# zuds-survey/zuds-pipeline

Hardware: AMD Instinct MI355X
Metric: Mpix/s resample->coadd->subtract, 3072x3072 frames (higher is better)
Workload: dtype f32; 1 GPU; configs[1]+[2]: 32x 3072x3072 TPV frames/GPU, mesh background + weight rescale + Lanczos-3 resample + WEIGHTED coadd (+ AND mask coadd, int16 masks); then 1 science frame/GPU: align ref, hotpants 3x3 regions x 10x10 stamps, r=10, ko=4, subtract; frames_per_gpu=32, size=3072, mask_dtype=int16, combine=WEIGHTED, subtract=True

## Files before the change

### zuds-pipeline_amd/csrc/hotpants.hip

```cpp
#include "hp_dev.h"
#include <sched.h>
#include "chol_diag.h"

__global__ void k_hp_valid(const float* __restrict__ sci, const float* __restrict__ ref,
                           const uint8_t* __restrict__ bpm, int64_t n, float il, float iu,
                           float tl, float tu, uint8_t* __restrict__ bad,
                           const double* __restrict__ lim, double nsig) {
    int64_t p = (int64_t)blockIdx.x * blockDim.x + threadIdx.x;
    if (lim) {
        il = (float)(lim[0] - nsig * lim[1]);
        tl = (float)(lim[3] - nsig * lim[4]);
    }
    if (p >= n) return;
    float s = sci[p], t = ref[p];
    bool ok = (s == s) && (t == t) && fabsf(s) < 3e38f && fabsf(t) < 3e38f;
    ok = ok && s >= il && s <= iu && t >= tl && t <= tu;
    if (bpm) ok = ok && bpm[p] == 0;
    bad[p] = ok ? 0 : 1;
}

#define HP_ROWMAX 16384
__global__ __launch_bounds__(256) void k_hp_rowany(const uint8_t* __restrict__ in, int nx, int ny, int hw,
                                                   uint8_t* __restrict__ out) {
    extern __shared__ int ra_pre[];
// ... 1811 lines not shown
    if (tid < 64) {
        auto run_chain = [&](double* xout) {
            const int li = tid & 31;
            double col[CH_NB];
#pragma unroll
            for (int j = 0; j < CH_NB; ++j) col[j] = Dn[j][li];
            const double rdl = Dn[li][CH_NB];
            double u = ys[li];
#pragma unroll
            for (int j = 1; j < CH_NB; ++j) col[j] *= readlane_d(rdl, j);
#pragma unroll
            for (int j = CH_NB - 1; j >= 1; --j) u = __builtin_fma(-col[j], readlane_d(u, j), u);
            if (tid < CH_NB) xout[tid] = u * rdl;
        };
        __syncthreads();
        run_chain(xs[0]);
        __syncthreads();
        for (int kb = nblk - 1; kb >= 1; --kb) {
            __syncthreads();
            run_chain(xs[(nblk - kb) & 1]);
            __syncthreads();
        }
        return;
    }
    const int c = tid - 64;
    double yc = 0.0, a[CH_NB], dnext[2] = {0.0, 0.0};
    auto diag_elem = [&](int k0, int nb, int e) -> double {
        const int i = e >> 5, j = e & 31;
        return (i < nb && j <= i) ? A[(size_t)(k0 + i) * lda + k0 + j] : (i == j ? 1.0 : 0.0);
    };
    auto diag_put = [&](int e, double v) {
        const int i = e >> 5, j = e & 31;
        Dn[i][j] = (i == j) ? 0.0 : v;
        if (i == j) Dn[i][CH_NB] = 1.0 / v;
    };
    {
        const int kb = nblk - 1, k0 = kb * CH_NB, nb = n - k0;
        yc = (c < n) ? A[(size_t)n * lda + c] : 0.0;
        diag_put(c, diag_elem(k0, nb, c));
        if (c + CBC_COLS < CH_NB * CH_NB) diag_put(c + CBC_COLS, diag_elem(k0, nb, c + CBC_COLS));
        if (c >= k0 && c < k0 + CH_NB) ys[c - k0] = yc;
#pragma unroll
        for (int m = 0; m < CH_NB; ++m) a[m] = (c < k0 && m < nb) ? A[(size_t)(k0 + m) * lda + c] : 0.0;
        if (kb > 0) {
            dnext[0] = diag_elem(k0 - CH_NB, CH_NB, c);
            if (c + CBC_COLS < CH_NB * CH_NB) dnext[1] = diag_elem(k0 - CH_NB, CH_NB, c + CBC_COLS);
        }
    }
    __syncthreads();
    __syncthreads();
    for (int kb = nblk - 1; kb >= 1; --kb) {
        const int k0 = kb * CH_NB, nb = min(CH_NB, n - k0);
        const int k0n = k0 - CH_NB;
        const double* xc = xs[(nblk - 1 - kb) & 1];
        if (c >= k0 && c < k0 + nb) yc = xc[c - k0];
        if (c >= k0n && c < k0) {
            double acc = 0.0;
#pragma unroll
            for (int m = 0; m < CH_NB; ++m) acc += a[m] * xc[m];
            yc -= acc;
            ys[c - k0n] = yc;
        }
        diag_put(c, dnext[0]);
        if (c + CBC_COLS < CH_NB * CH_NB) diag_put(c + CBC_COLS, dnext[1]);
        __syncthreads();
        if (c < k0n) {
            double acc = 0.0;
#pragma unroll
            for (int m = 0; m < CH_NB; ++m) acc += a[m] * xc[m];
            yc -= acc;
        }
#pragma unroll
        for (int m = 0; m < CH_NB; ++m) a[m] = (c < k0n) ? A[(size_t)(k0n + m) * lda + c] : 0.0;
        if (kb > 1) {
            dnext[0] = diag_elem(k0n - CH_NB, CH_NB, c);
            if (c + CBC_COLS < CH_NB * CH_NB) dnext[1] = diag_elem(k0n - CH_NB, CH_NB, c + CBC_COLS);
        }
        __syncthreads();
    }
    if (c < min(CH_NB, n)) yc = xs[(nblk - 1) & 1][c];
    if (c < n) xall[(size_t)blockIdx.x * n + c] = yc / dall[(size_t)blockIdx.x * n + c];
}

static __device__ __forceinline__ void hp_merit_body(const hp_plan& P, const double* __restrict__ G,
                                                 const double* __restrict__ phi,
                                                 const double* __restrict__ vbar,
                                                 const int* __restrict__ active,
                                                 const double* __restrict__ xsol,
                                                 double* __restrict__ merit, const int* __restrict__ guard,
                                                 int* __restrict__ needlist) {
    if (guard && *guard == 0) return;
    __shared__ double c[HP_MAXX];
    const int cell = blockIdx.x, lane = threadIdx.x;
    if (needlist && cell == 0 && lane == 0) needlist[0] = 0;
    if (active[cell] < 0) { if (lane == 0) merit[cell] = -1.0; return; }
    const int reg = cell / P.ncellr;
    const double* x = xsol + (size_t)reg * P.nunk;
    const double* ph = phi + (size_t)cell * P.nkp;
    const double* Gc = G + (size_t)cell * HP_MAXX * HP_MAXX;
    if (lane < P.nE) {
        double v;
        if (lane == 0) v = x[0];
        else if (lane < P.nc) {
            v = 0.0;
            for (int p = 0; p < P.nkp; ++p) v += x[1 + (lane - 1) * P.nkp + p] * ph[p];
        } else v = x[1 + (P.nc - 1) * P.nkp + (lane - P.nc)];
        c[lane] = v;
    }
    __syncthreads();
    double part = 0.0;
    if (lane < P.nE) {
        double q = 0.0;
        for (int m = 0; m < P.nE; ++m) q += Gc[lane * HP_MAXX + m] * c[m];
        part = c[lane] * (q - 2.0 * Gc[lane * HP_MAXX + P.nE]);
    }
    part = wave_sum_d(part);
    if (lane == 0) merit[cell] = (Gc[P.nE * HP_MAXX + P.nE] + part) / (P.npix * vbar[cell]);
}

#define HP_RFLAG_TMO (1 << 30)
#define HP_RFLAG_DONE 0x80000000u
struct hp_sig {
    int* done;
    unsigned long long* host;
    unsigned seq;
};
static __device__ __forceinline__ void hp_round_signal(const hp_sig& sg, int* round_flag, int nblocks) {
    if (!sg.host) return;
    __threadfence();
    __syncthreads();
    if (threadIdx.x == 0 && atomicAdd(sg.done, 1) == nblocks - 1) {
        const unsigned v = (unsigned)atomicAdd(round_flag, 0);
        __threadfence_system();
        __hip_atomic_store(sg.host, ((unsigned long long)sg.seq << 32) | v | HP_RFLAG_DONE, __ATOMIC_RELEASE,
                           __HIP_MEMORY_SCOPE_SYSTEM);
    }
}
__global__ __launch_bounds__(256) void k_hp_reject(const hp_plan P, const double* __restrict__ merit,
                                                   const int2* __restrict__ centres,
                                                   int* __restrict__ active, int* __restrict__ need,
                                                   int* __restrict__ chg, int* __restrict__ nrej,
                                                   double* __restrict__ stats, const int* __restrict__ guard, int* __restrict__ round_flag,
                                                   int* __restrict__ needlist, const int* __restrict__ tmo = nullptr,
                                                   const hp_sig sig = hp_sig{nullptr, nullptr, 0u}) {
    if (guard && *guard == 0) {
        hp_round_signal(sig, round_flag, gridDim.x);
        return;
    }
    __shared__ double red[4];
    const int reg = blockIdx.x, tid = threadIdx.x;
    double m = 0.0, s = 0.0;
    for (int pass = 0; pass < 4; ++pass) {
        double s0 = 0, s1 = 0;
        for (int k = tid; k < P.ncellr; k += 256) {
            double v = merit[reg * P.ncellr + k];
            if (active[reg * P.ncellr + k] < 0) continue;
            if (pass == 0 || fabs(v - m) <= 3.0 * s) { s0 += 1.0; s1 += v; }
        }
        s0 = block_sum256(s0, red);
        s1 = block_sum256(s1, red);
        if (s0 < 1.0) break;
        double mn = s1 / s0, s2 = 0;
        for (int k = tid; k < P.ncellr; k += 256) {
            double v = merit[reg * P.ncellr + k];
            if (active[reg * P.ncellr + k] < 0) continue;
            if (pass == 0 || fabs(v - m) <= 3.0 * s) s2 += (v - mn) * (v - mn);
        }
        s2 = block_sum256(s2, red);
        m = mn;
        s = sqrt(s2 / s0);
    }
    const double lim = m + P.ks * s;
    double cnt = 0, msum = 0, used = 0;
    for (int k = tid; k < P.ncellr; k += 256) {
        const int cell = reg * P.ncellr + k;
        int a = active[cell];
        need[cell] = 0;
        chg[cell] = 0;
        if (a < 0) continue;
        double v = merit[cell];
        used += 1.0;
        msum += v;
        if (v > lim) {
            cnt += 1.0;
            a += 1;
            if (a >= P.nss || centres[cell * P.nss + a].x < 0) a = -1;
            else {
                need[cell] = 1;
                if (needlist) needlist[1 + atomicAdd(&needlist[0], 1)] = cell;
            }
            active[cell] = a;
            chg[cell] = 1;
        }
    }
    cnt = block_sum256(cnt, red);
    msum = block_sum256(msum, red);
    used = block_sum256(used, red);
    if (tid == 0) {
        nrej[reg] = (int)cnt;
        if (cnt > 0) atomicAdd(round_flag, (int)cnt);
        if (tmo && tmo[reg]) atomicOr(round_flag, HP_RFLAG_TMO);
        stats[reg * 2 + 0] = used > 0 ? msum / used : 0.0;
        stats[reg * 2 + 1] = used;
    }
    __syncthreads();
    if (tid == 0) {
        int* list = chg + P.ncell + reg * (P.ncellr + 1);
        int k = 0;
        for (int c = 0; c < P.ncellr; ++c)
            if (chg[reg * P.ncellr + c]) list[1 + k++] = reg * P.ncellr + c;
        list[0] = k;
    }
    hp_round_signal(sig, round_flag, gridDim.x);
}

static __device__ __forceinline__ void hp_reject_wave_body(const hp_plan& P, const double* __restrict__ merit,
                                                       const int2* __restrict__ centres,
                                                       int* __restrict__ active, int* __restrict__ need,
                                                       int* __restrict__ chg, int* __restrict__ nrej,
                                                       double* __restrict__ stats, const int* __restrict__ guard,
                                                       int* __restrict__ round_flag, int* __restrict__ needlist,
                                                       const int* __restrict__ tmo = nullptr) {
    if (guard && *guard == 0) return;
    const int reg = blockIdx.x, lane = threadIdx.x;
    double mv[4];
    int av[4];
#pragma unroll
    for (int u = 0; u < 4; ++u) {
        const int k = lane + 64 * u;
        mv[u] = k < P.ncellr ? merit[reg * P.ncellr + k] : 0.0;
        av[u] = k < P.ncellr ? active[reg * P.ncellr + k] : -1;
    }
    double m = 0.0, s = 0.0;
    for (int pass = 0; pass < 4; ++pass) {
        double s0 = 0, s1 = 0;
#pragma unroll
        for (int u = 0; u < 4; ++u)
            if (av[u] >= 0 && (pass == 0 || fabs(mv[u] - m) <= 3.0 * s)) { s0 += 1.0; s1 += mv[u]; }
        s0 = wave_sum_d(s0);
        s1 = wave_sum_d(s1);
        if (s0 < 1.0) break;
        const double mn = s1 / s0;
        double s2 = 0;
#pragma unroll
        for (int u = 0; u < 4; ++u)
            if (av[u] >= 0 && (pass == 0 || fabs(mv[u] - m) <= 3.0 * s)) s2 += (mv[u] - mn) * (mv[u] - mn);
        s2 = wave_sum_d(s2);
        m = mn;
        s = sqrt(s2 / s0);
    }
    const double lim = m + P.ks * s;
    double cnt = 0, msum = 0, used = 0;
    unsigned long long chm[4];
#pragma unroll
    for (int u = 0; u < 4; ++u) {
        const int k = lane + 64 * u;
        bool changed = false;
        if (k < P.ncellr) {
            const int cell = reg * P.ncellr + k;
            int a = av[u];
            int nd = 0;
            if (a >= 0) {
                used += 1.0;
                msum += mv[u];
                if (mv[u] > lim) {
                    cnt += 1.0;
                    a += 1;
                    if (a >= P.nss || centres[cell * P.nss + a].x < 0) a = -1;
                    else nd = 1;
                    active[cell] = a;
                    changed = true;
                }
            }
            need[cell] = nd;
            chg[cell] = changed ? 1 : 0;
            if (nd && needlist) needlist[1 + atomicAdd(&needlist[0], 1)] = cell;
        }
        chm[u] = __ballot(changed);
    }
    cnt = wave_sum_d(cnt);
    msum = wave_sum_d(msum);
    used = wave_sum_d(used);
    if (lane == 0) {
        nrej[reg] = (int)cnt;
        if (cnt > 0) atomicAdd(round_flag, (int)cnt);
        if (tmo && tmo[reg]) atomicOr(round_flag, HP_RFLAG_TMO);
        stats[reg * 2 + 0] = used > 0 ? msum / used : 0.0;
        stats[reg * 2 + 1] = used;
    }
    int* list = chg + P.ncell + reg * (P.ncellr + 1);
    int base = 0;
#pragma unroll
    for (int u = 0; u < 4; ++u) {
        const unsigned long long bm = chm[u];
        if (bm >> lane & 1ull)
            list[1 + base + __popcll(bm & ((1ull << lane) - 1ull))] = reg * P.ncellr + lane + 64 * u;
        base += __popcll(bm);
    }
    if (lane == 0) list[0] = base;
}

__global__ void k_hp_init_active(const hp_plan P, const int2* __restrict__ centres,
                                 int* __restrict__ active, int* __restrict__ need,
                                 int* __restrict__ ntotal) {
    int cell = blockIdx.x * blockDim.x + threadIdx.x;
    if (cell >= P.ncell) return;
    bool has = centres[cell * P.nss].x >= 0;
    active[cell] = has ? 0 : -1;
    need[cell] = has ? 1 : 0;
    if (has) atomicAdd(&ntotal[cell / P.ncellr], 1);
}

__global__ __launch_bounds__(256) void k_hp_gram(const hp_plan P, const double* __restrict__ X,
// ... 72 lines not shown
}

__global__ void k_hp_scale(int n, int lda, const double* __restrict__ A0, const double* __restrict__ rhs0,
                           double* __restrict__ A, const double* __restrict__ d, unsigned* __restrict__ bar,
                           const int* __restrict__ guard, unsigned* __restrict__ dff, int ndff) {
    hp_scale_body(blockIdx.z, n, lda, A0, rhs0, A, d, bar, guard, dff, ndff);
}
#define HSB_ROWS 8
__global__ __launch_bounds__(256) void k_hp_scale_b(int n, int lda, int nreg, const hp_job* __restrict__ jobs, int round,
                                                    int ncell, int ncellr) {
    const hp_job& J = jobs[blockIdx.y / nreg];
    const int* guard = HPJ_GUARD(J, round);
    if (guard && *guard == 0) return;
    const int reg = blockIdx.y % nreg;
    if (HPJ_REGION_IDLE(J, round, reg, ncell, ncellr)) return;
    const double* __restrict__ dd = J.dsc + (size_t)reg * n;
    const double* __restrict__ A0 = J.A0 + (size_t)reg * (size_t)(n + 1) * n;
    const double* __restrict__ rhs0 = J.rhs0 + (size_t)reg * n;
    double* __restrict__ A = J.A + (size_t)reg * (size_t)(n + 1) * lda;
#pragma unroll 1
    for (int k = 0; k < HSB_ROWS; ++k) {
        const int c1 = blockIdx.x * HSB_ROWS + k;
        if (c1 >= n) break;
        const double r1 = 1.0 / dd[c1];
        for (int c2 = threadIdx.x; c2 <= c1; c2 += 256) {
            const double r2 = 1.0 / dd[c2];
            double v = __dmul_rn(A0[(size_t)c1 * n + c2], __dmul_rn(r1, r2));
            if (c1 == c2) v = __dadd_rn(v, HP_RIDGE);
            A[(size_t)c1 * lda + c2] = v;
        }
        if (threadIdx.x == 0) A[(size_t)n * lda + c1] = __dmul_rn(rhs0[c1], r1);
    }
}

__global__ __launch_bounds__(CT_THREADS) void k_chol_tp(int n, int lda, int ldt, double* Aall, double* ATall, int* fail,
                                                        long long* prof, const int* __restrict__ guard) {
    chol_tp_body(n, lda, ldt, Aall, ATall, fail, prof, guard);
}
__global__ __launch_bounds__(CT_THREADS) void k_chol_tp_b(int n, int lda, int ldt, const hp_job* __restrict__ jobs, int round,
                                                          int ncell, int ncellr) {
    const hp_job& J = jobs[blockIdx.z];
    if (HPJ_REGION_IDLE(J, round, (int)blockIdx.x, ncell, ncellr)) return;
    chol_tp_body(n, lda, ldt, J.A, J.AT, HPJ_FAIL(J), nullptr, HPJ_GUARD(J, round));
}

__global__ __launch_bounds__(CBC_THREADS) void k_chol_back_cols(int n, int lda, const double* __restrict__ Aall,
                                                                const double* __restrict__ dall,
                                                                double* __restrict__ xall, const int* __restrict__ guard) {
    chol_back_cols_body(n, lda, Aall, dall, xall, guard);
}
__global__ __launch_bounds__(CBC_THREADS) void k_chol_back_cols_b(int n, int lda, const hp_job* __restrict__ jobs, int round,
                                                                  int ncell, int ncellr) {
    const hp_job& J = jobs[blockIdx.z];
    if (HPJ_REGION_IDLE(J, round, (int)blockIdx.x, ncell, ncellr)) return;
    chol_back_cols_body(n, lda, J.A, J.dsc, J.rhs, HPJ_GUARD(J, round));
}

__global__ __launch_bounds__(64) void k_hp_merit(const hp_plan P, const double* __restrict__ G,
                                                 const double* __restrict__ phi, const double* __restrict__ vbar,
                                                 const int* __restrict__ active, const double* __restrict__ xsol,
                                                 double* __restrict__ merit, const int* __restrict__ guard,
                                                 int* __restrict__ needlist) {
    hp_merit_body(P, G, phi, vbar, active, xsol, merit, guard, needlist);
}
__global__ __launch_bounds__(64) void k_hp_merit_b(const hp_plan P, const hp_job* __restrict__ jobs, int round) {
    const hp_job& J = jobs[blockIdx.z];
    hp_merit_body(P, J.G, J.phi, J.vbar, J.active, J.rhs, J.merit, HPJ_GUARD(J, round), J.needlist);
}

__global__ __launch_bounds__(64) void k_hp_reject_wave(const hp_plan P, const double* __restrict__ merit,
                                                       const int2* __restrict__ centres, int* __restrict__ active,
                                                       int* __restrict__ need, int* __restrict__ chg,
                                                       int* __restrict__ nrej, double* __restrict__ stats,
                                                       const int* __restrict__ guard, int* __restrict__ round_flag,
                                                       int* __restrict__ needlist, const int* __restrict__ tmo,
                                                       const hp_sig sig) {
    hp_reject_wave_body(P, merit, centres, active, need, chg, nrej, stats, guard, round_flag, needlist, tmo);
    hp_round_signal(sig, round_flag, gridDim.x);
}
__global__ __launch_bounds__(64) void k_hp_reject_wave_b(const hp_plan P, const hp_job* __restrict__ jobs, int round) {
    const hp_job& J = jobs[blockIdx.z];
    hp_reject_wave_body(P, J.merit, J.centres, J.active, J.need, J.chg, HPJ_NREJ(J), J.stats, HPJ_GUARD(J, round),
                        J.rflags + round, J.needlist);
}

__global__ void k_hp_flag(int32_t* __restrict__ mask, const float* __restrict__ img, float value, int32_t bit,
                          int64_t n, const int* __restrict__ tmo, int nreg) {
    int gaveup = 0;
    for (int r = 0; r < nreg; ++r) gaveup |= tmo[r];
    if (gaveup) return;
    int64_t p = (int64_t)blockIdx.x * blockDim.x + threadIdx.x;
    if (p >= n) return;
    if (img[p] == value) mask[p] |= bit;
}

extern "C" void zm_hp_params_default(zm_hp_params* p) {
    if (!p) return;
    memset(p, 0, sizeof(*p));
    p->tu = 5e3; p->tl = 0.0; p->iu = 5e3; p->il = 0.0;
    p->r = 10.0; p->rss = 15.0;
    p->fin = sqrt(50000.0); p->fi = 1e-30;
    p->nsx = p->nsy = 10; p->nrx = p->nry = 1;
    p->ko = 4; p->bgo = 0; p->nss = 3; p->normalize = 0;
    p->ft = 20.0; p->ks = 2.0;
    p->ngauss = 3;
    p->deg[0] = 6; p->deg[1] = 4; p->deg[2] = 2;
    p->sigma[0] = 0.7; p->sigma[1] = 1.5; p->sigma[2] = 3.0;
    p->limits_dev = nullptr; p->limits_nsigma = 10.0;
}

static int make_plan(const zm_hp_params* hp, int nx, int ny, hp_plan* P, std::vector<double>* filt,
                     std::vector<double>* basis) {
    memset(P, 0, sizeof(*P));
    P->nx = nx; P->ny = ny;
    P->hwk = (int)hp->r; P->hwss = (int)hp->rss;
    ZM_CHECK(P->hwk >= 1 && P->hwk <= HP_MAX_HWK, "zm_subtract: kernel half width int(r) = %d outside [1, %d]", P->hwk, HP_MAX_HWK);
    ZM_CHECK(P->hwss >= 1 && P->hwss <= HP_MAX_HWSS, "zm_subtract: substamp half width int(rss) = %d outside [1, %d]", P->hwss, HP_MAX_HWSS);
    P->hw = P->hwk + P->hwss;
    P->step = 2 * P->hwk + 1; P->sw = 2 * P->hwss + 1; P->pw = 2 * P->hw + 1;
    P->npix = P->sw * P->sw;
    P->npixp = (P->npix + GR_KT - 1) / GR_KT * GR_KT;
    ZM_CHECK(hp->ngauss >= 1 && hp->ngauss <= 4, "zm_subtract: ngauss %d outside [1, 4]", hp->ngauss);
    ZM_CHECK(hp->ko >= 0 && hp->ko <= 6, "zm_subtract: -ko %d outside [0, 6]", hp->ko);
    ZM_CHECK(hp->bgo >= 0 && hp->bgo <= 3, "zm_subtract: -bgo %d outside [0, 3]", hp->bgo);
    ZM_CHECK(hp->nss >= 1 && hp->nss <= HP_MAXNSS, "zm_subtract: nss %d outside [1, %d]", hp->nss, HP_MAXNSS);
    ZM_CHECK(hp->nrx >= 1 && hp->nry >= 1 && hp->nrx * hp->nry <= HP_MAXREG, "zm_subtract: bad -nrx/-nry");
    ZM_CHECK(hp->nsx >= 1 && hp->nsy >= 1 && hp->nsx * hp->nsy <= 4096, "zm_subtract: bad -nsx/-nsy");
    P->ko = hp->ko; P->bgo = hp->bgo; P->nss = hp->nss; P->normalize = hp->normalize;
    P->nrx = hp->nrx; P->nry = hp->nry; P->nsx = hp->nsx; P->nsy = hp->nsy;
    P->nreg = hp->nrx * hp->nry; P->ncellr = hp->nsx * hp->nsy; P->ncell = P->nreg * P->ncellr;
    P->tu = hp->tu; P->tl = hp->tl; P->iu = hp->iu; P->il = hp->il; P->ft = hp->ft; P->ks = hp->ks;
    P->fi = (float)hp->fi; P->fin = (float)hp->fin;
    ZM_CHECK(nx / hp->nrx / hp->nsx >= 1 && ny / hp->nry / hp->nsy >= 1, "zm_subtract: stamps smaller than a pixel");
    for (int ry = 0; ry < hp->nry; ++ry)
        for (int rx = 0; rx < hp->nrx; ++rx) {
            int r = ry * hp->nrx + rx;
            P->rx0[r] = rx * (nx / hp->nrx);
            P->rx1[r] = rx == hp->nrx - 1 ? nx : (rx + 1) * (nx / hp->nrx);
            P->ry0[r] = ry * (ny / hp->nry);
            P->ry1[r] = ry == hp->nry - 1 ? ny : (ry + 1) * (ny / hp->nry);
        }
    const int step = P->step, hwk = P->hwk;
    std::vector<int> fidx;
    int nf1 = 0, nc = 0;
    std::vector<double> fsum;
    filt->clear();
    int base[4] = {0, 0, 0, 0};
    for (int g = 0; g < hp->ngauss; ++g) {
        ZM_CHECK(hp->deg[g] >= 0 && hp->deg[g] <= 8 && hp->sigma[g] > 0, "zm_subtract: bad basis");
        base[g] = nf1;
        P->gdeg[g] = hp->deg[g];
        P->gbase[g] = nf1;
        for (int a = 0; a <= hp->deg[g]; ++a) {
            double s = 0.0;
            for (int u = -hwk; u <= hwk; ++u) {
                double v = exp(-(double)u * u / (2.0 * hp->sigma[g] * hp->sigma[g])) * pow((double)u, (double)a);
                filt->push_back(v);
                s += v;
            }
            fsum.push_back(s);
            ++nf1;
        }
    }
    ZM_CHECK(nf1 <= HP_MAXF1, "zm_subtract: too many 1-D filters");
    P->nf1 = nf1;
    P->ngauss = hp->ngauss;
// ... 189 lines not shown
    ZM_TRY(ctx->get("hp_bad", np, (void**)&bad));
    ZM_TRY(ctx->get("hp_tmp8", np, (void**)&tmp8));
    ZM_TRY(ctx->get("hp_dirty", np, (void**)&dirty));
    ZM_TRY(ctx->get("hp_outbad", np, (void**)&outbad));
    int2* centres = nullptr;
    int *active = nullptr, *need = nullptr, *ibuf = nullptr;
    double *X = nullptr, *G = nullptr, *phi = nullptr, *vbar = nullptr, *A = nullptr, *rhs = nullptr,
           *dsc = nullptr, *merit = nullptr, *stats = nullptr, *d_filt = nullptr;
    ZM_TRY(ctx->get("hp_centres", sizeof(int2) * P.ncell * P.nss, (void**)&centres));
    ZM_TRY(ctx->get("hp_active", sizeof(int) * P.ncell, (void**)&active));
    ZM_TRY(ctx->get("hp_need", sizeof(int) * P.ncell, (void**)&need));
    int* needlist = nullptr;
    ZM_TRY(ctx->get("hp_needlist", sizeof(int) * ((size_t)P.ncell + 1), (void**)&needlist));
    int* chg = nullptr;
    ZM_TRY(ctx->get("hp_chg", sizeof(int) * (2 * (size_t)P.ncell + P.nreg), (void**)&chg));
    constexpr int HP_NIBUF = 4 * HP_MAXREG + 4;
    constexpr size_t HP_SUMBYTES = sizeof(int) * HP_NIBUF + sizeof(double) * 3 * HP_MAXREG;
    static_assert((sizeof(int) * HP_NIBUF) % 8 == 0, "the statistics behind the counters are doubles");
    char* sumbuf = nullptr;
    ZM_TRY(ctx->get("hp_summary", HP_SUMBYTES, (void**)&sumbuf));
    ibuf = reinterpret_cast<int*>(sumbuf);
    int *nrej = ibuf, *ntotal = ibuf + HP_MAXREG, *fail = ibuf + 2 * HP_MAXREG, *nmasked = ibuf + 3 * HP_MAXREG;
    int* tmo = ibuf + 3 * HP_MAXREG + 4;
    unsigned* cbar = nullptr;
    ZM_TRY(ctx->get("hp_cbar", sizeof(unsigned) * CF_BAR_STRIDE * HP_MAXREG, (void**)&cbar));
    double* cdg = nullptr;
    ZM_TRY(ctx->get("hp_cdg", sizeof(double) * 4 * CH_NB * (CH_NB + 1) * HP_MAXREG, (void**)&cdg));
    ZM_TRY(ctx->get("hp_X", sizeof(double) * (size_t)P.ncell * P.nX * P.npixp, (void**)&X));
    ZM_TRY(ctx->get("hp_G", sizeof(double) * (size_t)P.ncell * HP_MAXX * HP_MAXX, (void**)&G));
    double* Gp = nullptr;
    ZM_TRY(ctx->get("hp_Gp", sizeof(double) * (size_t)P.ncell * GR_SPLIT * HP_MAXX * HP_MAXX, (void**)&Gp));
    ZM_TRY(ctx->get("hp_phi", sizeof(double) * (size_t)P.ncell * P.nkp, (void**)&phi));
    double *Gold = nullptr, *phiold = nullptr;
    ZM_TRY(ctx->get("hp_Gold", sizeof(double) * (size_t)P.ncell * HP_MAXX * HP_MAXX, (void**)&Gold));
    ZM_TRY(ctx->get("hp_phiold", sizeof(double) * (size_t)P.ncell * P.nkp, (void**)&phiold));
    ZM_TRY(ctx->get("hp_vbar", sizeof(double) * P.ncell, (void**)&vbar));
    const int lda = (P.nunk + 15) & ~15;
    ZM_TRY(ctx->get("hp_A", sizeof(double) * (size_t)P.nreg * (P.nunk + 1) * lda, (void**)&A));
    ZM_TRY(ctx->get("hp_rhs", sizeof(double) * (size_t)P.nreg * P.nunk, (void**)&rhs));
    double *A0 = nullptr, *rhs0 = nullptr;
    ZM_TRY(ctx->get("hp_A0", sizeof(double) * (size_t)P.nreg * (P.nunk + 1) * P.nunk, (void**)&A0));
    ZM_TRY(ctx->get("hp_rhs0", sizeof(double) * (size_t)P.nreg * P.nunk, (void**)&rhs0));
    ZM_TRY(ctx->get("hp_dsc", sizeof(double) * (size_t)P.nreg * P.nunk, (void**)&dsc));
    ZM_TRY(ctx->get("hp_merit", sizeof(double) * P.ncell, (void**)&merit));
    stats = reinterpret_cast<double*>(sumbuf + sizeof(int) * HP_NIBUF);
    double* x0sum = stats + 2 * HP_MAXREG;
    ZM_TRY(ctx->get("hp_filt", sizeof(double) * filt.size(), (void**)&d_filt));
    if (!(ctx->hp_filt_dev == (const void*)d_filt && ctx->hp_filt_host == filt)) {
        double* h_tab = nullptr;
        ZM_TRY(ctx->get_pinned("hp_tab", sizeof(double) * filt.size(), (void**)&h_tab));
        ZM_HIP(hipStreamSynchronize(st));
        memcpy(h_tab, filt.data(), sizeof(double) * filt.size());
        ZM_HIP(hipMemcpyAsync(d_filt, h_tab, sizeof(double) * filt.size(), hipMemcpyHostToDevice, st));
        ctx->hp_filt_host = filt;
        ctx->hp_filt_dev = d_filt;
    }

    const dim3 b256(256);
    ZM_TRY(hp_launch_masks(ctx, P, hp, sci, ref, bpm, bad, tmp8, dirty, outbad));
    char* h_sum = nullptr;
    ZM_TRY(ctx->get_pinned("hp_summary_h", HP_SUMBYTES, (void**)&h_sum));
    const int* h_int = reinterpret_cast<const int*>(h_sum);
    const double* h_stats = reinterpret_cast<const double*>(h_sum + sizeof(int) * HP_NIBUF);
    const double* h_x0 = h_stats + 2 * HP_MAXREG;
    int rounds = 0, retries = 0, ntimeouts = 0;
    const char* spin_env = getenv("ZM_CHOL_SPIN_LIMIT");
    hp_fit_guard fitting(&g_hp_fitting[ctx->device & 63]);
    for (int attempt = 0; attempt < 2; ++attempt) {
    const bool safe = attempt > 0;
    const int spin_limit = (!safe && spin_env) ? atoi(spin_env) : CF_SPIN_LIMIT;
    ZM_HIP(hipMemsetAsync(ibuf, 0, sizeof(int) * HP_NIBUF, st));
    ZM_TRY(hp_launch_cells(ctx, P, ref, bad, dirty, centres, active, need, ntotal));
    const hv_cfg hvc = hp_vectors_cfg(P.pw, P.sw, P.npix);
    ZM_CHECK(hvc.cw >= 8, "zm_subtract: r = %d, rss = %d: the template patch alone exceeds the LDS", P.hwk, P.hwss);
    size_t vsh = hvc.shmem;
    const int hv_gx = hvc.big ? std::min(P.ncell, 128) : P.ncell;
    double* hv_w0g = nullptr;
    if (hvc.w0_global)
        ZM_TRY(ctx->get("hp_w0g", sizeof(double) * (size_t)hv_gx * HV_SPLIT_FEW * P.npix, (void**)&hv_w0g));

    int* rflags = nullptr;
    int* h_rflags = nullptr;
    hipEvent_t* evs = nullptr;
    ZM_TRY(ctx->get("hp_rflags", sizeof(int) * 32, (void**)&rflags));
    ZM_TRY(ctx->get_pinned("hp_rflags_h", sizeof(int) * 16, (void**)&h_rflags));
    ZM_TRY(zm_get_sync_events(ctx, 3, &evs));
    ZM_HIP(hipMemsetAsync(rflags, 0, sizeof(int) * 32, st));
    if (!ctx->hp_sig_h) {
        ZM_HIP(hipHostMalloc((void**)&ctx->hp_sig_h, sizeof(unsigned long long) * 16, hipHostMallocCoherent | hipHostMallocMapped));
        memset(ctx->hp_sig_h, 0, sizeof(unsigned long long) * 16);
        ZM_HIP(hipHostGetDevicePointer((void**)&ctx->hp_sig_d, ctx->hp_sig_h, 0));
    }
    static const bool sig_off = ZM_DEVENV("ZM_HP_SIGNAL") && ZM_DEVENV("ZM_HP_SIGNAL")[0] == '0';
    const unsigned seq = ++ctx->hp_seq;
    auto enqueue_round = [&](const int rounds) -> int {
        const int* guard = rounds > 1 ? rflags + (rounds - 1) : nullptr;
        const int ncl_grid = std::min(P.ncell, 48);
        if (rounds > 1) {
            zm_scope_timer t(ctx, "hp_solve");
            int nt = zm_div_up(P.nunk, 16);
            if (P.nkp > 16)
                hipLaunchKernelGGL(k_hp_build, dim3(nt, nt, P.nreg), b256, 0, st, P, G, phi, active, chg, -1, A0, rhs0, guard);
        }
        {
            zm_scope_timer t(ctx, "hp_vectors");
            ZM_TRY(zm_hp_launch_vectors(ctx, st, P, hvc, rounds, ncl_grid, hv_gx, sci, ref, sci_rms, ref_rms, d_filt, centres, active,
                                        need, X, phi, vbar, guard, phiold, needlist, hv_w0g));
            ZM_HIP(hipGetLastError());
        }
        {
            zm_scope_timer t(ctx, "hp_gram");
            hipLaunchKernelGGL(k_hp_gram, dim3(rounds == 1 ? P.ncell : ncl_grid, GR_SPLIT), b256, 0, st, P, X, need, active, Gp, guard,
                               rounds == 1 ? nullptr : needlist);
            hipLaunchKernelGGL(k_hp_gram_sum, dim3(rounds == 1 ? P.ncell : ncl_grid), dim3(GS_THREADS), 0, st, Gp, need, active, G, guard, Gold,
                               rounds == 1 ? nullptr : needlist);
            ZM_HIP(hipGetLastError());
        }
        {
            zm_scope_timer t(ctx, "hp_solve");
            int nt = zm_div_up(P.nunk, 16);
            const char* form_env = getenv("ZM_CHOL_FORM");
            bool tp = safe || ctx->share >= 2 || fitting.shared();
            if (form_env && !strcmp(form_env, "tp")) tp = true;
            if (form_env && (!strcmp(form_env, "lat") || !strcmp(form_env, "df")) && !safe) tp = false;
            if (!ctx->hp_wg_cap) {
                int occ = 0, ncu = 0;
                ZM_HIP(hipOccupancyMaxActiveBlocksPerMultiprocessor(&occ, (const void*)k_chol_fused, 256, 0));
                ZM_HIP(hipDeviceGetAttribute(&ncu, hipDeviceAttributeMultiprocessorCount, ctx->device));
                ctx->hp_wg_cap = std::max(1, std::min(occ, 1) * (ncu - ncu / 16));
                if (ZM_DEVENV("ZM_CHOL_PROF")) fprintf(stderr, "chol: occupancy %d x %d CUs\n", occ, ncu);
            }
            const int wg_cap = ctx->hp_wg_cap / std::max(ctx->share, 1);
            const int W = std::max(2, std::min(68, wg_cap / P.nreg));
            const int nunk = P.nunk;
            static const bool want_prof = ZM_DEVENV("ZM_CHOL_PROF") && atoi(ZM_DEVENV("ZM_CHOL_PROF")) != 0;
            const bool want_df = !tp && !(form_env && !strcmp(form_env, "lat")) && 2 * P.nreg <= wg_cap && W <= 128;
            const int ndff = hp_df_nflags(P.nunk);
            unsigned* dff = nullptr;
            double* dfdg = nullptr;
            int* dftiles = nullptr;
            bool df = want_df;
            if (df) {
                constexpr int TW = 1 + 2 * DF_MAXT;
                int* htl = nullptr;
                ZM_TRY(ctx->get_pinned("hp_dftiles_h", sizeof(int) * (3 + 128 * TW), (void**)&htl));
                ZM_TRY(ctx->get("hp_dftiles", sizeof(int) * 128 * TW, (void**)&dftiles));
                constexpr int DF_MAGIC = 0x64663031;
                const bool known = htl[2] == DF_MAGIC && htl[1] == W && (htl[0] == nunk || htl[0] == -nunk - 1);
                if (!known) {
                    ZM_HIP(hipStreamSynchronize(st));
                    bool fits = true;
                    for (int wg = 0; wg < W; ++wg) {
                        int ti[DF_MAXT] = {0, 0, 0}, tj[DF_MAXT] = {0, 0, 0}, ntl = 0;
                        fits = hp_df_owner(nunk, W, wg, ti, tj, &ntl) && fits;
                        htl[3 + wg * TW] = ntl;
                        for (int k = 0; k < DF_MAXT; ++k) { htl[3 + wg * TW + 1 + 2 * k] = ti[k]; htl[3 + wg * TW + 2 + 2 * k] = tj[k]; }
                    }
                    htl[0] = fits ? nunk : -nunk - 1;
                    htl[1] = W;
                    htl[2] = DF_MAGIC;
                    if (fits) ZM_HIP(hipMemcpyAsync(dftiles, htl + 3, sizeof(int) * W * TW, hipMemcpyHostToDevice, st));
                }
                df = htl[0] == nunk;
            }
            if (df) {
                ZM_TRY(ctx->get("hp_dfflags", sizeof(unsigned) * (size_t)ndff * P.nreg, (void**)&dff));
                ZM_TRY(ctx->get("hp_dfdg", sizeof(double) * (size_t)P.nreg * zm_div_up(P.nunk, CH_NB) * CH_NB * (CH_NB + 1),
                                (void**)&dfdg));
            }
            static const bool build_scalar = ZM_DEVENV("ZM_BUILD_FORM") && !strcmp(ZM_DEVENV("ZM_BUILD_FORM"), "scalar");
// ... 24 lines not shown
                        hipLaunchKernelGGL(k_chol_tp, dim3(P.nreg), dim3(CT_THREADS), 0, st, P.nunk, lda, ldt, A, AT, fail, parg, guard);
                    }
                    ZM_HIP(hipGetLastError());
                    if (tp_prof) {
                        std::vector<long long> hp((size_t)5 * P.nreg);
                        ZM_HIP(hipMemcpyAsync(hp.data(), parg, sizeof(long long) * hp.size(), hipMemcpyDeviceToHost, st));
                        ZM_HIP(hipStreamSynchronize(st));
                        static const char* nm[5] = {"init", "products", "diag", "factor", "solve"};
                        fprintf(stderr, "chol_tp wg 0:");
                        for (int k = 0; k < 5; ++k) fprintf(stderr, " %s %.1f us", nm[k], hp[k] * 0.01);
                        fprintf(stderr, "\n");
                    }
                } else {
                ZM_CHECK(2 * P.nreg <= wg_cap,
                         "zm_subtract: %d regions exceed the %d resident workgroups of this context's share (1 / %d)",
                         P.nreg, wg_cap, ctx->share);
                const int nprof = df ? 8 : 6;
                long long* parg = nullptr;
                const int nblkp = zm_div_up(nunk, CH_NB);
                if (want_prof) ZM_TRY(ctx->get("hp_cprof", sizeof(long long) * 8 * ((size_t)P.nreg * W + (size_t)P.nreg * nblkp), (void**)&parg));
                {
                    zm_scope_timer tc(ctx, "hp_chol");
                    if (df) {
                        static const int prof_mode = want_prof ? std::min(2, atoi(ZM_DEVENV("ZM_CHOL_PROF"))) : 0;
#ifdef ZM_DEV
                        auto kf = prof_mode == 2 ? k_chol_df<2> : prof_mode == 1 ? k_chol_df<1> : k_chol_df<0>;
#else
                        auto kf = k_chol_df<0>;
#endif
                        static bool df_attr[3][64] = {};
                        if (!df_attr[prof_mode][ctx->device & 63]) {
                            ZM_HIP(hipFuncSetAttribute((const void*)kf, hipFuncAttributeMaxDynamicSharedMemorySize,
                                                       (int)sizeof(df_lds)));
                            df_attr[prof_mode][ctx->device & 63] = true;
                        }
                        hipLaunchKernelGGL(kf, dim3(P.nreg * W), dim3(DF_THREADS), sizeof(df_lds), st, nunk, lda, W, A,
                                           dfdg, fail, tmo, spin_limit, dff, dftiles, guard, A0, rhs0, dsc, parg);
                    } else {
                        hipLaunchKernelGGL(k_chol_fused, dim3(P.nreg * W), b256, 0, st, nunk, lda, W, A, cdg, fail, tmo,
                                           spin_limit, cbar, parg, guard);
                    }
                }
                ZM_HIP(hipGetLastError());
                if (want_prof) {
                    std::vector<long long> hp((size_t)8 * ((size_t)P.nreg * W + (size_t)P.nreg * nblkp));
                    ZM_HIP(hipMemcpyAsync(hp.data(), parg, sizeof(long long) * hp.size(), hipMemcpyDeviceToHost, st));
                    ZM_HIP(hipStreamSynchronize(st));
                    static const char* nm6[6] = {"load", "tilewait", "panel", "barrier1", "update", "barrier2"};
                    static const char* nm8[8] = {"load", "flagwait", "coeff", "factor", "publish", "solve", "panels", "update"};
                    const int NCd = (nunk + 63) / 64;
                    std::vector<int> show = {0, 1, W - 1, W, (P.nreg - 1) * W};
                    if (df) show = {0, 1, NCd / 2, NCd - 1, std::min(NCd, W - 1), W - 1, (P.nreg - 1) * W + 1};
                    for (int wg : show) {
                        fprintf(stderr, "chol wg %3d:", wg);
                        for (int k = 0; k < nprof; ++k)
                            fprintf(stderr, " %s %.1f us", df ? nm8[k] : nm6[k], hp[(size_t)wg * nprof + k] * 0.01);
                        fprintf(stderr, "\n");
                    }
                    if (df && ZM_DEVENV("ZM_CHOL_PROF") && atoi(ZM_DEVENV("ZM_CHOL_PROF")) >= 2) {
                        const long long* ts = hp.data() + (size_t)8 * P.nreg * W;
                        for (int kb = 0; kb < nblkp; ++kb) {
                            fprintf(stderr, "chol kb %2d:", kb);
                            for (int e = 0; e < 6; ++e) fprintf(stderr, " %7.2f", (ts[kb * 8 + e] - ts[0]) * 0.01);
                            fprintf(stderr, "\n");
                        }
                    }
                }
                }
            }
            {
                const size_t bsh = sizeof(double) * (((size_t)P.nunk + 1) & ~(size_t)1) +
                                   sizeof(double) * CH_NB * (CH_NB + 1);
                if (!ctx->hp_bset && bsh > 65536) {
                    ZM_HIP(hipFuncSetAttribute((const void*)k_chol_back,
                                               hipFuncAttributeMaxDynamicSharedMemorySize, 160 * 1024 - 64));
                    ctx->hp_bset = true;
                }
                ZM_CHECK(bsh <= 160 * 1024 - 64, "zm_subtract: %d unknowns exceed the solver's LDS", P.nunk);
                if (P.nunk <= CBC_COLS)
                    hipLaunchKernelGGL(k_chol_back_cols, dim3(P.nreg), dim3(CBC_THREADS), 0, st, P.nunk, lda, A, dsc, rhs, guard);
                else
                    hipLaunchKernelGGL(k_chol_back, dim3(P.nreg), dim3(1024), bsh, st, P.nunk, lda, A, dsc, rhs, guard);
            }
            hipLaunchKernelGGL(k_hp_merit, dim3(P.ncell), dim3(64), 0, st, P, G, phi, vbar, active, rhs, merit, guard, needlist);
            const hp_sig sig = sig_off ? hp_sig{nullptr, nullptr, 0u} : hp_sig{rflags + 16 + rounds, ctx->hp_sig_d + rounds, seq};
            if (P.ncellr <= 256)
                hipLaunchKernelGGL(k_hp_reject_wave, dim3(P.nreg), dim3(64), 0, st, P, merit, centres, active, need,
                                   chg, nrej, stats, guard, rflags + rounds, needlist, (const int*)tmo, sig);
            else
                hipLaunchKernelGGL(k_hp_reject, dim3(P.nreg), b256, 0, st, P, merit, centres, active, need, chg,
                                   nrej, stats, guard, rflags + rounds, needlist, (const int*)tmo, sig);
            ZM_HIP(hipGetLastError());
        }
        if (sig_off) {
            ZM_HIP(hipMemcpyAsync(h_rflags + rounds, rflags + rounds, sizeof(int), hipMemcpyDeviceToHost, st));
            ZM_HIP(hipEventRecord(evs[1 + (rounds & 1)], st));
        }
        return 0;
    };
    auto wait_round = [&](int r, int* flag) -> int {
        if (sig_off) {
            ZM_HIP(hipEventSynchronize(evs[1 + (r & 1)]));
            *flag = h_rflags[r];
            return 0;
        }
        for (unsigned long spins = 1;; ++spins) {
            const unsigned long long w = __atomic_load_n(&ctx->hp_sig_h[r], __ATOMIC_ACQUIRE);
            if ((unsigned)(w >> 32) == seq && ((unsigned)w & HP_RFLAG_DONE)) {
                *flag = (int)((unsigned)w & ~HP_RFLAG_DONE);
                return 0;
            }
            if ((spins & 0x3ffff) == 0) {
                const hipError_t e = hipStreamQuery(st);
                if (e == hipSuccess) {
                    const unsigned long long w2 = __atomic_load_n(&ctx->hp_sig_h[r], __ATOMIC_ACQUIRE);
                    ZM_CHECK((unsigned)(w2 >> 32) == seq && ((unsigned)w2 & HP_RFLAG_DONE),
                             "zm_subtract: round %d finished without signalling the host", r);
                } else if (e != hipErrorNotReady) {
                    ZM_HIP(e);
                }
            }
            if (spins < 4096) __builtin_ia32_pause();
            else sched_yield();
        }
    };
    rounds = 0;
    ZM_TRY(enqueue_round(1));
    bool tmo_seen = false;
    for (int r = 1; r <= 8; ++r) {
        if (r < 8) ZM_TRY(enqueue_round(r + 1));
        int flag = 0;
        ZM_TRY(wait_round(r, &flag));
        rounds = r;
        tmo_seen = tmo_seen || (flag & HP_RFLAG_TMO);
        if ((flag & ~HP_RFLAG_TMO) == 0 || tmo_seen) break;
    }
    {
        zm_scope_timer t(ctx, "hp_apply");
        unsigned long long* smask = nullptr;
        ZM_TRY(ctx->get("hp_smask", sizeof(unsigned long long), (void**)&smask));
        hipLaunchKernelGGL(k_hp_solved, dim3(1), dim3(64), 0, st, P.nreg, P.nunk, stats, fail, tmo, rhs, smask, x0sum);
        {
            ZM_TRY(zm_hp_launch_apply(ctx, P, smask, sci, ref, sci_rms, ref_rms, outbad, d_filt, rhs, out_diff, out_rms, nmasked));
        }
    }
    if (hp->flag_mask_dev) {
        hipLaunchKernelGGL(k_hp_flag, dim3((unsigned)((np + 255) / 256)), b256, 0, st, hp->flag_mask_dev, out_diff, 1e-30f,
                           hp->flag_bit, np, tmo, P.nreg);
        ZM_HIP(hipGetLastError());
    }
    ZM_HIP(hipMemcpyAsync(h_sum, sumbuf, HP_SUMBYTES, hipMemcpyDeviceToHost, st));
    if (hp->async_info && !tmo_seen) {
        if (!ctx->hp_done) ZM_HIP(hipEventCreateWithFlags(&ctx->hp_done, hipEventDisableTiming));
        ZM_HIP(hipEventRecord(ctx->hp_done, st));
        ctx->hp_pending = true;
        ctx->hp_pend_rounds = rounds;
        ctx->hp_pend_retries = retries;
        ctx->hp_pend_nreg = P.nreg;
        ctx->hp_pend_nunk = P.nunk;
        fitting.release();
        if (info) {
            memset(info, 0, sizeof(*info));
            info->status = ZM_HP_PENDING;
            info->niter = rounds;
            info->ncoeff = P.nunk;
            info->retries = retries;
        }
        return 0;
    }
    ZM_HIP(hipStreamSynchronize(st));
    ntimeouts = 0;
    for (int reg = 0; reg < P.nreg; ++reg) ntimeouts += h_int[3 * HP_MAXREG + 4 + reg];
    if (ntimeouts == 0) break;
    if (!safe) {
// ... 332 lines not shown
```

Before: 49260 Mpix/s.

## Fuse hotpants merit and reject kernels via last-block-per-region completion counter

Replaces the separate merit kernel and per-region reject kernel with one kernel. Each cell block computes its merit, bumps a per-region atomic counter, and the last block of each region runs the sigma-clipping rejection. Merit values go through shared-coherent stores and loads. This removes one kernel launch and the grid-wide barrier per rejection round, at the cost of atomics, a spin-wait on the needlist reset, and a larger flag buffer that must be zeroed.

```diff
diff --git a/zuds-pipeline_amd/csrc/hotpants.hip b/zuds-pipeline_amd/csrc/hotpants.hip
--- a/zuds-pipeline_amd/csrc/hotpants.hip
+++ b/zuds-pipeline_amd/csrc/hotpants.hip
@@ -1917,6 +1917,7 @@
     if (c < n) xall[(size_t)blockIdx.x * n + c] = yc / dall[(size_t)blockIdx.x * n + c];
 }
 
+template <bool SH = false>
 static __device__ __forceinline__ void hp_merit_body(const hp_plan& P, const double* __restrict__ G,
                                                  const double* __restrict__ phi,
                                                  const double* __restrict__ vbar,
@@ -1928,7 +1929,10 @@
     __shared__ double c[HP_MAXX];
     const int cell = blockIdx.x, lane = threadIdx.x;
     if (needlist && cell == 0 && lane == 0) needlist[0] = 0;
-    if (active[cell] < 0) { if (lane == 0) merit[cell] = -1.0; return; }
+    if (active[cell] < 0) {
+        if (lane == 0) { if (SH) st_sh(merit + cell, -1.0); else merit[cell] = -1.0; }
+        return;
+    }
     const int reg = cell / P.ncellr;
     const double* x = xsol + (size_t)reg * P.nunk;
     const double* ph = phi + (size_t)cell * P.nkp;
@@ -1950,11 +1954,18 @@
         part = c[lane] * (q - 2.0 * Gc[lane * HP_MAXX + P.nE]);
     }
     part = wave_sum_d(part);
-    if (lane == 0) merit[cell] = (Gc[P.nE * HP_MAXX + P.nE] + part) / (P.npix * vbar[cell]);
+    if (lane == 0) {
+        const double v = (Gc[P.nE * HP_MAXX + P.nE] + part) / (P.npix * vbar[cell]);
+        if (SH) st_sh(merit + cell, v); else merit[cell] = v;
+    }
 }
 
 #define HP_RFLAG_TMO (1 << 30)
 #define HP_RFLAG_DONE 0x80000000u
+#define HP_RFLAG_WORDS 32
+#define HP_MR_PAD 32
+#define HP_MR_SET ((HP_MAXREG + 1) * HP_MR_PAD)
+#define HP_RFLAG_INTS (HP_RFLAG_WORDS + 9 * HP_MR_SET)
 struct hp_sig {
     int* done;
     unsigned long long* host;
@@ -2049,21 +2060,22 @@
     hp_round_signal(sig, round_flag, gridDim.x);
 }
 
+template <bool SH = false>
 static __device__ __forceinline__ void hp_reject_wave_body(const hp_plan& P, const double* __restrict__ merit,
                                                        const int2* __restrict__ centres,
                                                        int* __restrict__ active, int* __restrict__ need,
                                                        int* __restrict__ chg, int* __restrict__ nrej,
                                                        double* __restrict__ stats, const int* __restrict__ guard,
                                                        int* __restrict__ round_flag, int* __restrict__ needlist,
-                                                       const int* __restrict__ tmo = nullptr) {
+                                                       const int* __restrict__ tmo = nullptr, int region = -1) {
     if (guard && *guard == 0) return;
-    const int reg = blockIdx.x, lane = threadIdx.x;
+    const int reg = region < 0 ? (int)blockIdx.x : region, lane = threadIdx.x;
     double mv[4];
     int av[4];
 #pragma unroll
     for (int u = 0; u < 4; ++u) {
         const int k = lane + 64 * u;
-        mv[u] = k < P.ncellr ? merit[reg * P.ncellr + k] : 0.0;
+        mv[u] = k < P.ncellr ? (SH ? ld_sh(merit + reg * P.ncellr + k) : merit[reg * P.ncellr + k]) : 0.0;
         av[u] = k < P.ncellr ? active[reg * P.ncellr + k] : -1;
     }
     double m = 0.0, s = 0.0;
@@ -2302,6 +2314,36 @@
     const hp_job& J = jobs[blockIdx.z];
     hp_reject_wave_body(P, J.merit, J.centres, J.active, J.need, J.chg, HPJ_NREJ(J), J.stats, HPJ_GUARD(J, round),
                         J.rflags + round, J.needlist);
+}
+
+__global__ __launch_bounds__(64) void k_hp_merit_reject(const hp_plan P, const double* __restrict__ G,
+                                                        const double* __restrict__ phi, const double* __restrict__ vbar,
+                                                        int* active, const double* __restrict__ xsol, double* merit,
+                                                        const int2* __restrict__ centres, int* need, int* chg,
+                                                        int* __restrict__ nrej, double* __restrict__ stats,
+                                                        const int* __restrict__ guard, int* round_flag, int* needlist,
+                                                        const int* __restrict__ tmo, const hp_sig sig, int* cnt) {
+    if (guard && *guard == 0) {
+        if (blockIdx.x == 0) hp_round_signal(sig, round_flag, 1);
+        return;
+    }
+    const int cell = blockIdx.x, reg = cell / P.ncellr;
+    hp_merit_body<true>(P, G, phi, vbar, active, xsol, merit, guard, nullptr);
+    __shared__ int last;
+    if (threadIdx.x == 0) {
+        if (cell == 0 && needlist)
+            __hip_atomic_store(needlist, 0, __ATOMIC_RELAXED, __HIP_MEMORY_SCOPE_AGENT);
+        asm volatile("s_waitcnt vmcnt(0)" ::: "memory");
+        if (cell == 0 && needlist) __hip_atomic_store(cnt + HP_MAXREG * HP_MR_PAD, 1, __ATOMIC_RELAXED, __HIP_MEMORY_SCOPE_AGENT);
+        last = __hip_atomic_fetch_add(cnt + reg * HP_MR_PAD, 1, __ATOMIC_RELAXED, __HIP_MEMORY_SCOPE_AGENT) == P.ncellr - 1;
+    }
+    __syncthreads();
+    if (!last) return;
+    if (needlist)
+        while (__hip_atomic_load(cnt + HP_MAXREG * HP_MR_PAD, __ATOMIC_RELAXED, __HIP_MEMORY_SCOPE_AGENT) == 0) __builtin_amdgcn_s_sleep(1);
+    asm volatile("" ::: "memory");
+    hp_reject_wave_body<true>(P, merit, centres, active, need, chg, nrej, stats, guard, round_flag, needlist, tmo, reg);
+    hp_round_signal(sig, round_flag, P.nreg);
 }
 
 __global__ void k_hp_flag(int32_t* __restrict__ mask, const float* __restrict__ img, float value, int32_t bit,
@@ -2657,10 +2699,10 @@
     int* rflags = nullptr;
     int* h_rflags = nullptr;
     hipEvent_t* evs = nullptr;
-    ZM_TRY(ctx->get("hp_rflags", sizeof(int) * 32, (void**)&rflags));
+    ZM_TRY(ctx->get("hp_rflags", sizeof(int) * HP_RFLAG_INTS, (void**)&rflags));
     ZM_TRY(ctx->get_pinned("hp_rflags_h", sizeof(int) * 16, (void**)&h_rflags));
     ZM_TRY(zm_get_sync_events(ctx, 3, &evs));
-    ZM_HIP(hipMemsetAsync(rflags, 0, sizeof(int) * 32, st));
+    ZM_HIP(hipMemsetAsync(rflags, 0, sizeof(int) * HP_RFLAG_INTS, st));
     if (!ctx->hp_sig_h) {
         ZM_HIP(hipHostMalloc((void**)&ctx->hp_sig_h, sizeof(unsigned long long) * 16, hipHostMallocCoherent | hipHostMallocMapped));
         memset(ctx->hp_sig_h, 0, sizeof(unsigned long long) * 16);
@@ -2851,14 +2893,21 @@
                 else
                     hipLaunchKernelGGL(k_chol_back, dim3(P.nreg), dim3(1024), bsh, st, P.nunk, lda, A, dsc, rhs, guard);
             }
-            hipLaunchKernelGGL(k_hp_merit, dim3(P.ncell), dim3(64), 0, st, P, G, phi, vbar, active, rhs, merit, guard, needlist);
             const hp_sig sig = sig_off ? hp_sig{nullptr, nullptr, 0u} : hp_sig{rflags + 16 + rounds, ctx->hp_sig_d + rounds, seq};
-            if (P.ncellr <= 256)
-                hipLaunchKernelGGL(k_hp_reject_wave, dim3(P.nreg), dim3(64), 0, st, P, merit, centres, active, need,
-                                   chg, nrej, stats, guard, rflags + rounds, needlist, (const int*)tmo, sig);
-            else
-                hipLaunchKernelGGL(k_hp_reject, dim3(P.nreg), b256, 0, st, P, merit, centres, active, need, chg,
-                                   nrej, stats, guard, rflags + rounds, needlist, (const int*)tmo, sig);
+            static const bool tail_split = ZM_DEVENV("ZM_HP_TAIL") && !strcmp(ZM_DEVENV("ZM_HP_TAIL"), "split");
+            if (P.ncellr <= 256 && !tail_split) {
+                hipLaunchKernelGGL(k_hp_merit_reject, dim3(P.ncell), dim3(64), 0, st, P, G, phi, vbar, active, rhs, merit, centres,
+                                   need, chg, nrej, stats, guard, rflags + rounds, needlist, (const int*)tmo, sig,
+                                   rflags + HP_RFLAG_WORDS + rounds * HP_MR_SET);
+            } else {
+                hipLaunchKernelGGL(k_hp_merit, dim3(P.ncell), dim3(64), 0, st, P, G, phi, vbar, active, rhs, merit, guard, needlist);
+                if (P.ncellr <= 256)
+                    hipLaunchKernelGGL(k_hp_reject_wave, dim3(P.nreg), dim3(64), 0, st, P, merit, centres, active, need,
+                                       chg, nrej, stats, guard, rflags + rounds, needlist, (const int*)tmo, sig);
+                else
+                    hipLaunchKernelGGL(k_hp_reject, dim3(P.nreg), b256, 0, st, P, merit, centres, active, need, chg,
+                                       nrej, stats, guard, rflags + rounds, needlist, (const int*)tmo, sig);
+            }
             ZM_HIP(hipGetLastError());
         }
         if (sig_off) {
```

New measurement: 49250 Mpix/s (median of 5 runs). No clear change (-0.0%).
